# bernardomig/torch_semantic_segmentation

Hardware: AMD Instinct MI355X
Metric: images/sec (train step) fastscnn 1024x2048 bs=8 (higher is better)
Workload: dtype bf16; 1 GPU; fastscnn train step (zero_grad+fwd+CE(ignore 255)+bwd+AdamW), 8 x 3 x 1024 x 2048 per GPU, 19 classes, random-init weights; global_batch=8, parallelism=dp1, hip_graph=True, syncbn=False

## Files before the change

### torch_semantic_segmentation_amd/csrc/wgrad.hip

```cpp
#include "common.h"
#include "wgreduce.h"
#include "bnfin.h"

extern int g_tss_disable_fast;

namespace {

constexpr int TN = 128, TK = 128, NT = 256;
enum { A_PW = 0, A_TAPS = 1, A_STEM = 2 };

template <typename T> struct WMma;
template <> struct WMma<bf16_t> {
  static constexpr int PT = 64, KSTEP = 32;
  typedef bf16x8 Frag;
  static __device__ __forceinline__ Frag ld(const unsigned char* row, int swz, int ks, int q) {
    return *reinterpret_cast<const bf16x8*>(row + (((ks * 4 + q) ^ swz) << 4));
  }
  static __device__ __forceinline__ f32x4 mma(Frag a, Frag b, f32x4 c) {
    return __builtin_amdgcn_mfma_f32_16x16x32_bf16(a, b, c, 0, 0, 0);
  }
};
template <> struct WMma<float> {
  static constexpr int PT = 32, KSTEP = 4;
  typedef float Frag;
  static __device__ __forceinline__ Frag ld(const unsigned char* row, int swz, int ks, int q) {
    return *reinterpret_cast<const float*>(row + ((ks ^ swz) << 4) + q * 4);
  }
  static __device__ __forceinline__ f32x4 mma(Frag a, Frag b, f32x4 c) {
    return __builtin_amdgcn_mfma_f32_16x16x4f32(a, b, c, 0, 0, 0);
  }
};
constexpr int ROWB = 144;

struct WgradArgs {
  long P;
  int ND, KD, ntaps, mode;
  const void* e; long lde; const void* yraw; long ldyr;
  const float* ga; const float* gb; const float* gce; const float* gmu;
  const void* x; long ldx; const float* xm; const float* xs; const float* xb; int x_relu, x_f32;
  int Hin, Win, Hout, Wout, stride, dil, Cin;
  int tap0, tstep1;
  int gkh, gkw;
  float* dw; long drs, dcs, dts;
  int nsplit;
  float* ws;
  tss_bn_bwd_job fin; int fin_blocks;
};

template <typename T> struct Pack4;
template <> struct Pack4<bf16_t> {
  static __device__ __forceinline__ void put(unsigned char* dst, float a, float b, float c, float d) {
    bf16x4 o; o[0] = (bf16_t)a; o[1] = (bf16_t)b; o[2] = (bf16_t)c; o[3] = (bf16_t)d;
    *reinterpret_cast<bf16x4*>(dst) = o;
  }
};
template <> struct Pack4<float> {
  static __device__ __forceinline__ void put(unsigned char* dst, float a, float b, float c, float d) {
    *reinterpret_cast<float4*>(dst) = make_float4(a, b, c, d);
  }
};
template <typename T>
__device__ __forceinline__ unsigned char* unit_addr(unsigned char* tile, int row, int pg) {
  const int boff = pg * 4 * (int)sizeof(T);
  return tile + row * ROWB + ((((boff >> 4)) ^ ((row >> 3) & 7)) << 4) + (boff & 15);
}
template <typename T>
__device__ __forceinline__ void put_unit(unsigned char* tile, int ch0, int pg, const float v[4][8]) {
#pragma unroll
  for (int j = 0; j < 8; ++j) Pack4<T>::put(unit_addr<T>(tile, ch0 + j, pg), v[0][j], v[1][j], v[2][j], v[3][j]);
}

template <typename T>
__global__ __launch_bounds__(NT, 2) void wgrad_kernel(const WgradArgs g) {
  typedef WMma<T> M;
  constexpr int PT = M::PT, NPG = PT / 4;
  constexpr bool FOLD = sizeof(T) == 2;
  __shared__ __align__(16) unsigned char Gt[TN * ROWB];
  __shared__ __align__(16) unsigned char At[TK * ROWB];
  __shared__ __align__(16) float Cg[4][TN];
  __shared__ __align__(16) float Ca[3][TK];

  const int tid = threadIdx.x, lane = tid & 63, wave = tid >> 6;
  const int fr = lane & 15, fq = lane >> 4;
  const int wn = wave >> 1, wk = wave & 1;

  const int nchn = (g.ND + TN - 1) / TN, nchk = (g.KD + TK - 1) / TK;
  int bid = blockIdx.x;
  const int split = bid % g.nsplit; bid /= g.nsplit;
  const int nc = bid % nchn; bid /= nchn;
  const int kc = bid % nchk; bid /= nchk;
  const int tap = bid;

  const int n0 = nc * TN, k0 = kc * TK;
  const int ncw = (g.ND - n0 < TN) ? (g.ND - n0) : TN;
  const int kcw = (g.KD - k0 < TK) ? (g.KD - k0) : TK;
  const int nvn = (ncw + 7) >> 3, nvk = (kcw + 7) >> 3;
  int nfn = (ncw - wn * 64 + 15) >> 4; nfn = nfn < 0 ? 0 : (nfn > 4 ? 4 : nfn);
  int nfk = (kcw - wk * 64 + 15) >> 4; nfk = nfk < 0 ? 0 : (nfk > 4 ? 4 : nfk);

  const long nstage = (g.P + PT - 1) / PT;
  const long per = (nstage + g.nsplit - 1) / g.nsplit;
  const long s_begin = split * per;
  long s_end = s_begin + per;
  if (s_end > nstage) s_end = nstage;

  f32x4 acc[4][4];
#pragma unroll
  for (int i = 0; i < 4; ++i)
#pragma unroll
    for (int j = 0; j < 4; ++j) acc[i][j] = (f32x4){0.f, 0.f, 0.f, 0.f};

  for (int i = tid; i < TN * ROWB / 16; i += NT) {
    reinterpret_cast<uint4*>(Gt)[i] = make_uint4(0, 0, 0, 0);
    reinterpret_cast<uint4*>(At)[i] = make_uint4(0, 0, 0, 0);
  }
  for (int i = tid; i < TN; i += NT) {
    const bool in = i < ncw;
    Cg[0][i] = (in && g.ga) ? g.ga[n0 + i] : 1.f;
    Cg[1][i] = (in && g.yraw) ? g.gb[n0 + i] : 0.f;
    Cg[2][i] = (in && g.yraw) ? g.gce[n0 + i] : 0.f;
    Cg[3][i] = (in && g.yraw) ? g.gmu[n0 + i] : 0.f;
    const bool ik = i < kcw && g.mode != A_STEM;
    Ca[0][i] = (ik && g.xs && g.xm) ? g.xm[k0 + i] : 0.f;
    Ca[1][i] = (ik && g.xs) ? g.xs[k0 + i] : 1.f;
    Ca[2][i] = (ik && g.xs && g.xb) ? g.xb[k0 + i] : 0.f;
  }

  const T* e = reinterpret_cast<const T*>(g.e);
  const T* yr = reinterpret_cast<const T*>(g.yraw);
  const T* x = reinterpret_cast<const T*>(g.x);
  const long HWo = (long)g.Hout * g.Wout;
  int tdy, tdx;
  if (g.gkw > 0) { const int ty = tap / g.gkw; tdy = ty - (g.gkh >> 1); tdx = (tap - ty * g.gkw) - (g.gkw >> 1); }
  else { const int tgrid = g.tap0 + tap * (g.tstep1 + 1); const int ky = tgrid / 3; tdy = ky - 1; tdx = tgrid - ky * 3 - 1; }
  tdy *= g.dil; tdx *= g.dil;

  for (long s = s_begin; s < s_end; ++s) {
    const long p0 = s * PT;
    __syncthreads();
    for (int u = tid; u < NPG * nvn; u += NT) {
      const int pg = u / nvn, cv = u - pg * nvn;
      const int ch = n0 + cv * 8;
      float v[4][8];
      float ca[8], cb[8], cc[8], cm[8];
#pragma unroll
      for (int j = 0; j < 8; ++j) {
        ca[j] = Cg[0][cv * 8 + j]; cb[j] = Cg[1][cv * 8 + j]; cc[j] = Cg[2][cv * 8 + j]; cm[j] = Cg[3][cv * 8 + j];
        if (FOLD) cc[j] = -(ca[j] * cc[j]) - cb[j] * cm[j];
      }
#pragma unroll
      for (int i = 0; i < 4; ++i) {
        const long p = p0 + pg * 4 + i;
        const bool ok = p < g.P;
        const long pc = ok ? p : 0;
        float ev[8];
        V8<T>::load(e + pc * g.lde + ch, ev);
        if (yr) {
          float yv[8];
          V8<T>::load(yr + pc * g.ldyr + ch, yv);
#pragma unroll
          for (int j = 0; j < 8; ++j)
            v[i][j] = FOLD ? ca[j] * ev[j] + (cb[j] * yv[j] + cc[j]) : ca[j] * (ev[j] - cc[j]) + cb[j] * (yv[j] - cm[j]);
        } else {
#pragma unroll
          for (int j = 0; j < 8; ++j) v[i][j] = ca[j] * ev[j];
        }
#pragma unroll
        for (int j = 0; j < 8; ++j) if (!ok || ch + j >= g.ND) v[i][j] = 0.f;
      }
      put_unit<T>(Gt, cv * 8, pg, v);
    }
    if (g.mode == A_STEM) {
      const float* src32 = reinterpret_cast<const float*>(g.x);
      for (int u = tid; u < NPG * kcw; u += NT) {
        const int pg = u % NPG, j = u / NPG;
        const int c = j / 9, t9 = j - c * 9, sy = t9 / 3, sx = t9 - sy * 3;
        float v[4];
#pragma unroll
        for (int i = 0; i < 4; ++i) {
          const long p = p0 + pg * 4 + i;
          v[i] = 0.f;
          if (p < g.P) {
            const long b = p / HWo; const long rem = p - b * HWo;
            const int oy = (int)(rem / g.Wout), ox = (int)(rem - (long)oy * g.Wout);
            const int iy = oy * g.stride + (sy - 1) * g.dil, ix = ox * g.stride + (sx - 1) * g.dil;
            if (iy >= 0 && iy < g.Hin && ix >= 0 && ix < g.Win) {
              const long off = ((b * g.Cin + c) * g.Hin + iy) * (long)g.Win + ix;
              v[i] = g.x_f32 ? src32[off] : (float)x[off];
            }
          }
        }
        Pack4<T>::put(unit_addr<T>(At, j, pg), v[0], v[1], v[2], v[3]);
      }
    } else {
      for (int u = tid; u < NPG * nvk; u += NT) {
        const int pg = u / nvk, cv = u - pg * nvk;
        const int ch = k0 + cv * 8;
        float v[4][8];
        float cm[8], cs[8], cb[8];
#pragma unroll
        for (int j = 0; j < 8; ++j) {
          cm[j] = Ca[0][cv * 8 + j]; cs[j] = Ca[1][cv * 8 + j]; cb[j] = Ca[2][cv * 8 + j];
          if (FOLD) cb[j] -= cm[j] * cs[j];
        }
#pragma unroll
        for (int i = 0; i < 4; ++i) {
          const long p = p0 + pg * 4 + i;
          long q = -1;
          if (p < g.P) {
            if (g.mode == A_PW) {
              q = p;
            } else {
              const long b = p / HWo; const long rem = p - b * HWo;
              const int oy = (int)(rem / g.Wout), ox = (int)(rem - (long)oy * g.Wout);
              const int iy = oy * g.stride + tdy, ix = ox * g.stride + tdx;
              if (iy >= 0 && iy < g.Hin && ix >= 0 && ix < g.Win) q = (b * g.Hin + iy) * (long)g.Win + ix;
            }
          }
          float xv[8];
          V8<T>::load(x + (q >= 0 ? q : 0) * g.ldx + ch, xv);
          const float vlo = q >= 0 ? (g.x_relu ? 0.f : -TSS_INF) : 0.f, vhi = q >= 0 ? TSS_INF : 0.f;
#pragma unroll
          for (int j = 0; j < 8; ++j) {
            v[i][j] = clamp3(FOLD ? xv[j] * cs[j] + cb[j] : (xv[j] - cm[j]) * cs[j] + cb[j], vlo, vhi);
            if (ch + j >= g.KD) v[i][j] = 0.f;
          }
        }
        put_unit<T>(At, cv * 8, pg, v);
      }
    }
    __syncthreads();
    if (nfn > 0 && nfk > 0) {
      const unsigned char* grow = Gt + (wn * 64 + fr) * ROWB;
      const unsigned char* arow = At + (wk * 64 + fr) * ROWB;
#pragma unroll
      for (int ks = 0; ks < PT / M::KSTEP; ++ks) {
        typename M::Frag gf[4], af[4];
#pragma unroll
        for (int i = 0; i < 4; ++i) {
          gf[i] = M::ld(grow + i * 16 * ROWB, ((wn * 64 + i * 16 + fr) >> 3) & 7, ks, fq);
          af[i] = M::ld(arow + i * 16 * ROWB, ((wk * 64 + i * 16 + fr) >> 3) & 7, ks, fq);
        }
#pragma unroll
        for (int i = 0; i < 4; ++i)
#pragma unroll
          for (int j = 0; j < 4; ++j)
            if (i < nfn && j < nfk) acc[i][j] = M::mma(gf[i], af[j], acc[i][j]);
      }
    }
  }

  float* dwt = g.dw + tap * g.dts;
  if (s_begin < s_end) {
#pragma unroll
    for (int i = 0; i < 4; ++i)
#pragma unroll
      for (int j = 0; j < 4; ++j) {
        if (i < nfn && j < nfk) {
          const int k = k0 + wk * 64 + j * 16 + fr;
#pragma unroll
          for (int r = 0; r < 4; ++r) {
            const int n = n0 + wn * 64 + i * 16 + fq * 4 + r;
            if (n < g.ND && k < g.KD) atomicAdd(dwt + (long)n * g.drs + (long)k * g.dcs, acc[i][j][r]);
          }
        }
      }
  }
}

using tss_wg::ws_dim;

#ifdef TSS_TIMING
__device__ unsigned long long g_wg_timing[8];
#define TSS_T(var) unsigned long long var; asm volatile("s_memtime %0\n s_waitcnt lgkmcnt(0)" : "=s"(var) :: "memory")
#else
#define TSS_T(var)
#endif
template <int PT>
__global__ __launch_bounds__(NT, 2) void wgfast_kernel(const WgradArgs g) {
  typedef bf16_t T;
  constexpr int NPG = PT / 4, ROW = PT * 2 + 16, NKS = PT / 32;
  TSS_T(tks);
  extern __shared__ __align__(16) unsigned char smem[];
  unsigned char* Gt = smem;
  unsigned char* At = smem + TN * ROW;

  const int tid = threadIdx.x, lane = tid & 63, wave = tid >> 6;
  const int fr = lane & 15, fq = lane >> 4;

  if ((int)blockIdx.x < g.fin_blocks) { tss_fin::bn_bwd_finalize_block(g.fin, blockIdx.x); return; }
  const int nchn = (g.ND + TN - 1) / TN;
  int bid = (int)blockIdx.x - g.fin_blocks;
  const int split = bid % g.nsplit; bid /= g.nsplit;
  const int nc = bid % nchn; bid /= nchn;
  const int kc = bid;
  const int n0 = nc * TN, k0 = kc * TK;
  const int ncw = (g.ND - n0 < TN) ? (g.ND - n0) : TN;
  const int kcw = (g.KD - k0 < TK) ? (g.KD - k0) : TK;
  const int nvn = ncw >> 3, nvk = kcw >> 3;
  const int FN = (ncw + 15) >> 4, FK = (kcw + 15) >> 4;

  int ib = 0, jb = 0, cn = 4, ck = 4, ks0 = 0, ks1 = NKS;
  if (FN > 4 && FK > 4) { ib = 4 * (wave >> 1); jb = 4 * (wave & 1); }
  else {
    ks0 = (wave & 1) * (NKS / 2); ks1 = ks0 + NKS / 2;
    if (FN > 4) ib = 4 * (wave >> 1);
    else if (FK > 4) jb = 4 * (wave >> 1);
    else if (FN > 2) { ib = 2 * (wave >> 1); cn = 2; }
    else { jb = 2 * (wave >> 1); ck = 2; }
  }
  cn = FN - ib < cn ? FN - ib : cn; cn = cn < 0 ? 0 : cn;
  ck = FK - jb < ck ? FK - jb : ck; ck = ck < 0 ? 0 : ck;

  const long nstage = (g.P + PT - 1) / PT;
  const long per = (nstage + g.nsplit - 1) / g.nsplit;
  const long s_begin = split * per;
  long s_end = s_begin + per;
  if (s_end > nstage) s_end = nstage;

  f32x4 acc[4][4];
#pragma unroll
  for (int i = 0; i < 4; ++i)
#pragma unroll
    for (int j = 0; j < 4; ++j) acc[i][j] = (f32x4){0.f, 0.f, 0.f, 0.f};

  const int pgG = tid / nvn, cvG = tid - pgG * nvn;
  const int pgA = tid / nvk, cvA = tid - pgA * nvk;
  const bool onG = pgG < NPG, onA = pgA < NPG;
  const T* eg = reinterpret_cast<const T*>(g.e) + n0 + (onG ? cvG * 8 : 0);
  const T* yg = reinterpret_cast<const T*>(g.yraw) + n0 + (onG ? cvG * 8 : 0);
  const T* xg = reinterpret_cast<const T*>(g.x) + k0 + (onA ? cvA * 8 : 0);
  uint4 re[4], ry[4], rx[4];
  auto issue_g = [&](long s) {
    const long p0 = s * PT;
    if (onG) {
#pragma unroll
      for (int i = 0; i < 4; ++i) {
        const long p = p0 + pgG * 4 + i;
        const long pc = p < g.P ? p : 0;
        re[i] = *reinterpret_cast<const uint4*>(eg + pc * g.lde);
        ry[i] = *reinterpret_cast<const uint4*>(yg + pc * g.ldyr);
      }
    }
  };
  auto issue_a = [&](long s) {
    const long p0 = s * PT;
    if (onA) {
#pragma unroll
      for (int i = 0; i < 4; ++i) {
        const long p = p0 + pgA * 4 + i;
        const long pc = p < g.P ? p : 0;
        rx[i] = *reinterpret_cast<const uint4*>(xg + pc * g.ldx);
      }
    }
  };
  auto unit_ptr = [&](unsigned char* tile, int row, int pg) -> unsigned char* {
    const int boff = pg * 8;
    return tile + row * ROW + ((((boff >> 4)) ^ ((row >> 3) & 7)) << 4) + (boff & 15);
  };
  auto blo = [](uint32_t u) { return __uint_as_float(u << 16); };
  auto bhi = [](uint32_t u) { return __uint_as_float(u & 0xffff0000u); };

#ifdef TSS_TIMING
  unsigned long long tph[7] = {0, 0, 0, 0, 0, 0, 0};
#endif
  if (s_begin < s_end) { issue_g(s_begin); issue_a(s_begin); }

  for (int i = tid; i < TN * ROW / 16; i += NT) {
    reinterpret_cast<uint4*>(Gt)[i] = make_uint4(0, 0, 0, 0);
    reinterpret_cast<uint4*>(At)[i] = make_uint4(0, 0, 0, 0);
  }
  float ca[8], cb[8], cc[8], as[8], ab[8];
  {
    const int chn = n0 + (onG ? cvG * 8 : 0), chk = k0 + (onA ? cvA * 8 : 0);
    const float* pxs = g.xs ? g.xs : g.ga;
    const float* pxb = (g.xs && g.xb) ? g.xb : g.ga;
    const float* pxm = (g.xs && g.xm) ? g.xm : g.ga;
    const int cks = g.xs ? chk : 0;
    float vga[8], vgb[8], vce[8], vmu[8], vs[8], vb[8], vm[8];
#pragma unroll
    for (int h = 0; h < 8; h += 4) {
      V4<float>::load(g.ga + chn + h, vga + h); V4<float>::load(g.gb + chn + h, vgb + h);
      V4<float>::load(g.gce + chn + h, vce + h); V4<float>::load(g.gmu + chn + h, vmu + h);
      V4<float>::load(pxs + cks + h, vs + h); V4<float>::load(pxb + cks + h, vb + h); V4<float>::load(pxm + cks + h, vm + h);
    }
    const bool has_s = g.xs != nullptr, has_b = has_s && g.xb != nullptr, has_m = has_s && g.xm != nullptr;
#pragma unroll
    for (int j = 0; j < 8; ++j) {
      ca[j] = vga[j]; cb[j] = vgb[j]; cc[j] = -(vga[j] * vce[j]) - vgb[j] * vmu[j];
      const float sc = has_s ? vs[j] : 1.f;
      as[j] = sc; ab[j] = (has_b ? vb[j] : 0.f) - (has_m ? vm[j] : 0.f) * sc;
    }
  }
  const float relu_lo = g.x_relu ? 0.f : -TSS_INF;
  TSS_T(tk1);
#ifdef TSS_TIMING
  tph[5] += tk1 - tks;
#endif
  for (long s = s_begin; s < s_end; ++s) {
    const long p0 = s * PT;
    TSS_T(t0);
    __syncthreads();
    TSS_T(t1);
    if (onG) {
      float v[4][8];
#pragma unroll
      for (int i = 0; i < 4; ++i) {
        const bool ok = p0 + pgG * 4 + i < g.P;
        const uint32_t* ue = reinterpret_cast<const uint32_t*>(&re[i]);
        const uint32_t* uy = reinterpret_cast<const uint32_t*>(&ry[i]);
#pragma unroll
        for (int h = 0; h < 4; ++h) {
          v[i][2 * h] = ca[2 * h] * blo(ue[h]) + (cb[2 * h] * blo(uy[h]) + cc[2 * h]);
          v[i][2 * h + 1] = ca[2 * h + 1] * bhi(ue[h]) + (cb[2 * h + 1] * bhi(uy[h]) + cc[2 * h + 1]);
        }
        if (!ok) {
#pragma unroll
          for (int j = 0; j < 8; ++j) v[i][j] = 0.f;
        }
      }
#pragma unroll
      for (int j = 0; j < 8; ++j) Pack4<T>::put(unit_ptr(Gt, cvG * 8 + j, pgG), v[0][j], v[1][j], v[2][j], v[3][j]);
    }
    TSS_T(t2);
    if (s + 1 < s_end) issue_g(s + 1);
    if (onA) {
      float v[4][8];
#pragma unroll
      for (int i = 0; i < 4; ++i) {
        const bool ok = p0 + pgA * 4 + i < g.P;
        const uint32_t* ux = reinterpret_cast<const uint32_t*>(&rx[i]);
#pragma unroll
        for (int h = 0; h < 4; ++h) {
          v[i][2 * h] = fmaxf(blo(ux[h]) * as[2 * h] + ab[2 * h], relu_lo);
          v[i][2 * h + 1] = fmaxf(bhi(ux[h]) * as[2 * h + 1] + ab[2 * h + 1], relu_lo);
        }
        if (!ok) {
#pragma unroll
          for (int j = 0; j < 8; ++j) v[i][j] = 0.f;
        }
      }
#pragma unroll
      for (int j = 0; j < 8; ++j) Pack4<T>::put(unit_ptr(At, cvA * 8 + j, pgA), v[0][j], v[1][j], v[2][j], v[3][j]);
    }
    if (s + 1 < s_end) issue_a(s + 1);
    TSS_T(t3);
    __syncthreads();
    TSS_T(t4);

    if (cn > 0 && ck > 0) {
      const int rg = ib * 16 + fr, rk = jb * 16 + fr;
      const unsigned char* grow = Gt + rg * ROW;
      const unsigned char* arow = At + rk * ROW;
      for (int ks = ks0; ks < ks1; ++ks) {
        bf16x8 gf[4], af[4];
#pragma unroll
        for (int i = 0; i < 4; ++i) {
          if (i < cn) gf[i] = *reinterpret_cast<const bf16x8*>(grow + i * 16 * ROW + (((ks * 4 + fq) ^ (((rg + i * 16) >> 3) & 7)) << 4));
          if (i < ck) af[i] = *reinterpret_cast<const bf16x8*>(arow + i * 16 * ROW + (((ks * 4 + fq) ^ (((rk + i * 16) >> 3) & 7)) << 4));
        }
#pragma unroll
        for (int i = 0; i < 4; ++i)
#pragma unroll
          for (int j = 0; j < 4; ++j)
            if (i < cn && j < ck) acc[i][j] = __builtin_amdgcn_mfma_f32_16x16x32_bf16(gf[i], af[j], acc[i][j], 0, 0, 0);
      }
    }
    TSS_T(t5);
#ifdef TSS_TIMING
    tph[0] += t1 - t0; tph[1] += t2 - t1; tph[2] += t3 - t2; tph[3] += t4 - t3; tph[4] += t5 - t4;
#endif
  }

  TSS_T(tkl);
  if (g.ws) {
    const bool psplit = !(FN > 4 && FK > 4);
    if (psplit) {
      __syncthreads();
      f32x4* xch = reinterpret_cast<f32x4*>(smem) + (wave >> 1) * 16 * 64;
      if (wave & 1) {
#pragma unroll
        for (int i = 0; i < 4; ++i)
#pragma unroll
          for (int j = 0; j < 4; ++j)
            if (i < cn && j < ck) xch[(i * 4 + j) * 64 + lane] = acc[i][j];
      }
      __syncthreads();
      if (!(wave & 1)) {
#pragma unroll
        for (int i = 0; i < 4; ++i)
#pragma unroll
          for (int j = 0; j < 4; ++j)
            if (i < cn && j < ck) acc[i][j] += xch[(i * 4 + j) * 64 + lane];
      }
    }
    if (!psplit || !(wave & 1)) {
      const int tile = kc * nchn + nc;
      const int TNe = ws_dim(g.ND), TKe = ws_dim(g.KD);
      float* wt = g.ws + ((long)tile * g.nsplit + split) * (TNe * TKe);
#pragma unroll
      for (int i = 0; i < 4; ++i)
#pragma unroll
        for (int j = 0; j < 4; ++j) {
          if (i < cn && j < ck) {
            float* wf = wt + ((ib + i) * (TKe >> 4) + (jb + j)) * 256 + fq * 16 + fr;
#pragma unroll
            for (int r = 0; r < 4; ++r) wf[r * 64] = acc[i][j][r];
          }
        }
    }
  } else if (s_begin < s_end) {
#pragma unroll
    for (int i = 0; i < 4; ++i)
#pragma unroll
      for (int j = 0; j < 4; ++j) {
        if (i < cn && j < ck) {
          const int k = k0 + (jb + j) * 16 + fr;
#pragma unroll
          for (int r = 0; r < 4; ++r) {
            const int n = n0 + (ib + i) * 16 + fq * 4 + r;
            if (n < g.ND && k < g.KD) atomicAdd(g.dw + (long)n * g.drs + (long)k * g.dcs, acc[i][j][r]);
          }
        }
      }
  }
#ifdef TSS_TIMING
  asm volatile("s_waitcnt vmcnt(0)" ::: "memory");
  TSS_T(tk2);
  tph[6] = tk2 - tkl;
  if (threadIdx.x == 0) {
    for (int q = 0; q < 7; ++q) atomicAdd(&g_wg_timing[q], tph[q]);
    atomicAdd(&g_wg_timing[7], 1ull);
  }
#endif
}

__global__ __launch_bounds__(NT) void wg_reduce_kernel(const tss_wg::ReduceArgs r) {
  __shared__ float4 part[4 * 64];
  tss_wg::reduce_block(r, blockIdx.x, part);
}

using tss_wg::reduce_args;

template <int PT>
void launch_fast_pt(WgradArgs& g, hipStream_t stream, bool defer_reduce) {
  const tss_wg::Split sp = tss_wg::split_for(g.P, g.KD, g.ND);
  g.nsplit = sp.nsplit;
  constexpr int smem = 2 * TN * (PT * 2 + 16);
  static tss::DevOnce attr;
  if (attr.first()) {
    (void)hipFuncSetAttribute(reinterpret_cast<const void*>(wgfast_kernel<PT>), hipFuncAttributeMaxDynamicSharedMemorySize, smem);
  }
  hipLaunchKernelGGL(wgfast_kernel<PT>, dim3(sp.tiles * g.nsplit + g.fin_blocks), dim3(NT), smem, stream, g);
  if (g.ws && !defer_reduce) {
    const tss_wg::ReduceArgs r = reduce_args(g.ws, g.dw, g.P, g.KD, g.ND);
    hipLaunchKernelGGL(wg_reduce_kernel, dim3(r.nred), dim3(NT), 0, stream, r);
  }
}

int launch(WgradArgs& g, int dtype, int kernel_id, hipStream_t stream, double alg_bytes) {
  if (g.P <= 0) return TSS_OK;
  const int nchn = (g.ND + TN - 1) / TN, nchk = (g.KD + TK - 1) / TK;
  const int tiles = nchn * nchk * g.ntaps;
  const int PT = dtype == TSS_BF16 ? WMma<bf16_t>::PT : WMma<float>::PT;
  const long nstage = (g.P + PT - 1) / PT;
  constexpr long MIN_STAGES = 8;
  long ns = 1024 / tiles;
  if (ns < 1) ns = 1;
  if (ns > (nstage + MIN_STAGES - 1) / MIN_STAGES) ns = (nstage + MIN_STAGES - 1) / MIN_STAGES;
  if (ns < 1) ns = 1;
  g.nsplit = (int)ns;
  const int grid = tiles * (int)ns;
  tss::ProfScope prof(kernel_id, stream, alg_bytes, 2.0 * (double)g.P * g.ND * g.KD * g.ntaps);
  if (dtype == TSS_BF16) hipLaunchKernelGGL(wgrad_kernel<bf16_t>, dim3(grid), dim3(NT), 0, stream, g);
  else hipLaunchKernelGGL(wgrad_kernel<float>, dim3(grid), dim3(NT), 0, stream, g);
  return tss::check_last("wgrad");
}

}

bool tss_stem_direct_wgrad(const void* e, long lde, const void* yraw, long ldyr, const float* ga, const float* gb,
                           const float* gce, const float* gmu, const void* x_nchw, int x_is_f32, float* dw, float* ws,
                           int B, int Cin, int Hin, int Win, int N, int stride, int dtype, hipStream_t stream);

void tss_wg_reduce_standalone(const float* ws, float* dw, long P, int K, int N, hipStream_t stream) {
  const tss_wg::ReduceArgs r = reduce_args(ws, dw, P, K, N);
  hipLaunchKernelGGL(wg_reduce_kernel, dim3(r.nred), dim3(NT), 0, stream, r);
}

extern "C" {

int tss_pwconv_bwd_weight(const void* e, long lde, const void* yraw, long ldyr,
                          const float* ga, const float* gb, const float* gce, const float* gmu,
                          const void* xraw, long ldx, const float* in_mean, const float* in_scale, const float* in_bias, int in_relu,
                          float* dw, float* ws, int defer_reduce, long P, int K, int N, int dtype, const tss_bn_bwd_job* fin,
                          void* stream) {
  TSS_REQUIRE(dtype == TSS_F32 || dtype == TSS_BF16, TSS_ERR_DTYPE);
  TSS_REQUIRE(!fin || (fin->C > 0 && fin->count >= 1.0 && fin->bstats && fin->invstd && fin->ga && fin->gb && fin->gce), TSS_ERR_SHAPE);
  TSS_REQUIRE(K > 0 && N > 0 && (K % 8) == 0 && (lde % 8) == 0 && lde >= (N + 7) / 8 * 8 && (ldx % 8) == 0 && ldx >= K, TSS_ERR_SHAPE);
  TSS_REQUIRE(!yraw || ((ldyr % 8) == 0 && ldyr >= (N + 7) / 8 * 8 && ga && gb && gce && gmu), TSS_ERR_SHAPE);
  TSS_REQUIRE(tss::aligned16(e) && tss::aligned16(xraw), TSS_ERR_ALIGN);
  WgradArgs g = {};
  g.P = P; g.ND = N; g.KD = K; g.ntaps = 1; g.mode = A_PW;
  g.e = e; g.lde = lde; g.yraw = yraw; g.ldyr = ldyr; g.ga = ga; g.gb = gb; g.gce = gce; g.gmu = gmu;
  g.x = xraw; g.ldx = ldx; g.xm = in_mean; g.xs = in_scale; g.xb = in_bias; g.x_relu = in_relu;
  g.Hout = 1; g.Wout = 1;
  g.dw = dw; g.drs = K; g.dcs = 1; g.dts = 0;
  const double bytes = (double)P * (N * (yraw ? 2 : 1) + K) * tss::esz(dtype);
  if (dtype == TSS_BF16 && !g_tss_disable_fast && yraw && (N % 8) == 0 && P > 0) {
    tss::ProfScope prof(TSS_K_PWCONV_BWD_WEIGHT, (hipStream_t)stream, bytes, 2.0 * (double)P * N * K);
    g.ws = ws;
    if (fin) { g.fin = *fin; g.fin_blocks = tss_fin::fin_blocks(fin->C); }
    if (tss_wg::split_for(P, K, N).pt == 128) launch_fast_pt<128>(g, (hipStream_t)stream, ws && defer_reduce);
    else launch_fast_pt<64>(g, (hipStream_t)stream, ws && defer_reduce);
    return tss::check_last("wgfast");
  }
  if (fin) {
    const int rc = tss_bn_bwd_finalize(fin->bstats, fin->count, fin->invstd, fin->gamma, fin->training, fin->accumulate, fin->dgamma,
                                       fin->dbeta, fin->ga, fin->gb, fin->gce, fin->C, stream);
    if (rc != TSS_OK) return rc;
  }
  return launch(g, dtype, TSS_K_PWCONV_BWD_WEIGHT, (hipStream_t)stream, bytes);
}

int tss_pwconv_wg_reduce(const float* ws, float* dw, long P, int K, int N, void* stream) {
  TSS_REQUIRE(ws && dw && P > 0 && K > 0 && N > 0 && (K % 8) == 0 && (N % 8) == 0, TSS_ERR_SHAPE);
  tss_wg_reduce_standalone(ws, dw, P, K, N, (hipStream_t)stream);
  return tss::check_last("wg_reduce");
}

long tss_pwconv_bwd_weight_ws(long P, int K, int N, int dtype) {
  if (dtype != TSS_BF16 || g_tss_disable_fast || (N % 8) != 0 || (K % 8) != 0 || P <= 0) return 0;
  const tss_wg::Split sp = tss_wg::split_for(P, K, N);
  return (long)sp.tiles * sp.nsplit * ws_dim(N) * ws_dim(K);
}

int tss_conv3x3_bwd_weight(const void* e, long lde, const void* yraw, long ldyr,
                           const float* ga, const float* gb, const float* gce, const float* gmu,
                           const void* xraw, long ldx, const float* in_mean, const float* in_scale, const float* in_bias, int in_relu,
                           float* dw, int B, int Hin, int Win, int Cin, int N, int stride, int dil,
                           int dtype, void* stream) {
  TSS_REQUIRE(dtype == TSS_F32 || dtype == TSS_BF16, TSS_ERR_DTYPE);
  TSS_REQUIRE(Cin > 0 && N > 0 && (Cin % 8) == 0 && (N % 8) == 0 && (lde % 8) == 0 && lde >= N && (ldx % 8) == 0 && ldx >= Cin,
              TSS_ERR_SHAPE);
  TSS_REQUIRE(!yraw || ((ldyr % 8) == 0 && ldyr >= N && ga && gb && gce && gmu), TSS_ERR_SHAPE);
  WgradArgs g = {};
  g.Hin = Hin; g.Win = Win; g.stride = stride; g.dil = dil; g.Cin = Cin;
  g.Hout = (Hin - 1) / stride + 1; g.Wout = (Win - 1) / stride + 1;
  g.P = (long)B * g.Hout * g.Wout; g.ND = N; g.KD = Cin; g.ntaps = 9; g.mode = A_TAPS;
  g.e = e; g.lde = lde; g.yraw = yraw; g.ldyr = ldyr; g.ga = ga; g.gb = gb; g.gce = gce; g.gmu = gmu;
  g.x = xraw; g.ldx = ldx; g.xm = in_mean; g.xs = in_scale; g.xb = in_bias; g.x_relu = in_relu;
  g.dw = dw; g.drs = (long)Cin * 9; g.dcs = 9; g.dts = 1;
  return launch(g, dtype, TSS_K_CONV3X3_BWD_WEIGHT, (hipStream_t)stream,
                ((double)g.P * N * (yraw ? 2 : 1) + (double)B * Hin * Win * Cin) * tss::esz(dtype));
}

int tss_conv1d3_bwd_weight(const void* e, long lde, const void* yraw, long ldyr,
                           const float* ga, const float* gb, const float* gce, const float* gmu,
                           const void* xraw, long ldx, const float* in_mean, const float* in_scale, const float* in_bias, int in_relu,
                           float* dw, int B, int H, int W, int Cin, int N, int axis, int dil, int dtype, void* stream) {
  TSS_REQUIRE(dtype == TSS_F32 || dtype == TSS_BF16, TSS_ERR_DTYPE);
  TSS_REQUIRE(Cin > 0 && N > 0 && (Cin % 8) == 0 && (N % 8) == 0 && (lde % 8) == 0 && lde >= N && (ldx % 8) == 0 && ldx >= Cin &&
              (axis == 0 || axis == 1) && dil >= 1, TSS_ERR_SHAPE);
  TSS_REQUIRE(!yraw || ((ldyr % 8) == 0 && ldyr >= N && ga && gb && gce && gmu), TSS_ERR_SHAPE);
  WgradArgs g = {};
  g.Hin = H; g.Win = W; g.stride = 1; g.dil = dil; g.Cin = Cin; g.Hout = H; g.Wout = W;
  g.tap0 = axis == 0 ? 3 : 1; g.tstep1 = axis == 0 ? 0 : 2;
  g.P = (long)B * H * W; g.ND = N; g.KD = Cin; g.ntaps = 3; g.mode = A_TAPS;
  g.e = e; g.lde = lde; g.yraw = yraw; g.ldyr = ldyr; g.ga = ga; g.gb = gb; g.gce = gce; g.gmu = gmu;
  g.x = xraw; g.ldx = ldx; g.xm = in_mean; g.xs = in_scale; g.xb = in_bias; g.x_relu = in_relu;
  g.dw = dw; g.drs = (long)Cin * 3; g.dcs = 3; g.dts = 1;
  return launch(g, dtype, TSS_K_CONV3X3_BWD_WEIGHT, (hipStream_t)stream,
                ((double)g.P * N * (yraw ? 2 : 1) + (double)g.P * Cin) * tss::esz(dtype));
}

int tss_convkxk_bwd_weight(const void* e, long lde, const void* yraw, long ldyr,
                           const float* ga, const float* gb, const float* gce, const float* gmu,
                           const void* xraw, long ldx, const float* in_mean, const float* in_scale, const float* in_bias, int in_relu,
                           float* dw, int B, int Hin, int Win, int Cin, int N, int kh, int kw, int stride, int dil,
                           int dtype, void* stream) {
  TSS_REQUIRE(dtype == TSS_F32 || dtype == TSS_BF16, TSS_ERR_DTYPE);
  TSS_REQUIRE(Cin > 0 && N > 0 && (Cin % 8) == 0 && (N % 8) == 0 && (lde % 8) == 0 && lde >= N && (ldx % 8) == 0 && ldx >= Cin &&
              stride >= 1 && dil >= 1 && kh >= 1 && kw >= 1 && (kh & 1) && (kw & 1) && kh * kw <= 81, TSS_ERR_SHAPE);
  TSS_REQUIRE(!yraw || ((ldyr % 8) == 0 && ldyr >= N && ga && gb && gce && gmu), TSS_ERR_SHAPE);
  WgradArgs g = {};
  g.Hin = Hin; g.Win = Win; g.stride = stride; g.dil = dil; g.Cin = Cin; g.gkh = kh; g.gkw = kw;
  g.Hout = (Hin - 1) / stride + 1; g.Wout = (Win - 1) / stride + 1;
  g.P = (long)B * g.Hout * g.Wout; g.ND = N; g.KD = Cin; g.ntaps = kh * kw; g.mode = A_TAPS;
  g.e = e; g.lde = lde; g.yraw = yraw; g.ldyr = ldyr; g.ga = ga; g.gb = gb; g.gce = gce; g.gmu = gmu;
  g.x = xraw; g.ldx = ldx; g.xm = in_mean; g.xs = in_scale; g.xb = in_bias; g.x_relu = in_relu;
  g.dw = dw; g.drs = (long)Cin * kh * kw; g.dcs = kh * kw; g.dts = 1;
  return launch(g, dtype, TSS_K_CONV3X3_BWD_WEIGHT, (hipStream_t)stream,
                ((double)g.P * N * (yraw ? 2 : 1) + (double)B * Hin * Win * Cin) * tss::esz(dtype));
}

int tss_stem3x3_bwd_weight(const void* e, long lde, const void* yraw, long ldyr,
                           const float* ga, const float* gb, const float* gce, const float* gmu,
                           const void* x_nchw, int x_is_f32, float* dw, float* ws,
                           int B, int Cin, int Hin, int Win, int N, int stride, int dtype, void* stream) {
  TSS_REQUIRE(dtype == TSS_F32 || dtype == TSS_BF16, TSS_ERR_DTYPE);
  TSS_REQUIRE(Cin >= 1 && Cin * 9 <= TK && N > 0 && (N % 8) == 0 && (lde % 8) == 0 && lde >= N, TSS_ERR_SHAPE);
  TSS_REQUIRE(!yraw || ((ldyr % 8) == 0 && ldyr >= N && ga && gb && gce && gmu), TSS_ERR_SHAPE);
  WgradArgs g = {};
  g.Hin = Hin; g.Win = Win; g.stride = stride; g.dil = 1; g.Cin = Cin;
  g.Hout = (Hin - 1) / stride + 1; g.Wout = (Win - 1) / stride + 1;
  g.P = (long)B * g.Hout * g.Wout; g.ND = N; g.KD = Cin * 9; g.ntaps = 1; g.mode = A_STEM;
  g.e = e; g.lde = lde; g.yraw = yraw; g.ldyr = ldyr; g.ga = ga; g.gb = gb; g.gce = gce; g.gmu = gmu;
  g.x = x_nchw; g.x_f32 = x_is_f32;
  g.dw = dw; g.drs = (long)Cin * 9; g.dcs = 1; g.dts = 0;
  const double bytes = (double)g.P * N * (yraw ? 2 : 1) * tss::esz(dtype) + (double)B * Cin * Hin * Win * (x_is_f32 ? 4 : tss::esz(dtype));
  if (dtype == TSS_BF16 && !g_tss_disable_fast && Cin <= 3 && N == 32 && ws) {
    tss::ProfScope prof(TSS_K_STEM_BWD_WEIGHT, (hipStream_t)stream, bytes, 2.0 * (double)g.P * N * Cin * 9);
    if (tss_stem_direct_wgrad(e, lde, yraw, ldyr, ga, gb, gce, gmu, x_nchw, x_is_f32, dw, ws, B, Cin, Hin, Win, N, stride,
                              dtype, (hipStream_t)stream))
      return tss::check_last("stem_direct_wgrad");
  }
  return launch(g, dtype, TSS_K_STEM_BWD_WEIGHT, (hipStream_t)stream, bytes);
}

#ifdef TSS_TIMING
int tss_debug_wg_timing(unsigned long long* out8, int reset) {
  if (hipMemcpyFromSymbol(out8, HIP_SYMBOL(g_wg_timing), sizeof(unsigned long long) * 8) != hipSuccess) return -1;
  if (reset) { unsigned long long z[8] = {0}; (void)hipMemcpyToSymbol(HIP_SYMBOL(g_wg_timing), z, sizeof(z)); }
  return 0;
}
#endif

}
```

Before: 1721 images/sec.

## Restructure wgrad fast kernel with row-major staging, transpose LDS reads and double buffering

Rewrites the pointwise-conv weight-gradient fast kernel. Threads now load whole rows and store them into a double-buffered LDS image, and MFMA operands come from transposed LDS reads (tr_pair). This replaces the old per-thread 4-pixel transpose-on-store into a single buffer. The kernel is fixed to 64-pixel sub-stages that iterate within the split's stage range, which removes the PT=128 variant. It also uses 32-bit unsigned offsets, so it adds a leading-dimension guard and falls back to the generic path when strides are large. The aim is fewer barriers per stage and cheaper LDS writes, at the cost of more shared memory and extra code from the template specialisations.

New measurement: 1728 images/sec (median of 6 runs). About the same (+0.4%).

```diff
diff --git a/torch_semantic_segmentation_amd/csrc/wgrad.hip b/torch_semantic_segmentation_amd/csrc/wgrad.hip
--- a/torch_semantic_segmentation_amd/csrc/wgrad.hip
+++ b/torch_semantic_segmentation_amd/csrc/wgrad.hip
@@ -1,5 +1,6 @@
 #include "common.h"
 #include "wgreduce.h"
+#include "wgsweep.h"
 #include "bnfin.h"
 
 extern int g_tss_disable_fast;
@@ -42,7 +43,7 @@
   int tap0, tstep1;
   int gkh, gkw;
   float* dw; long drs, dcs, dts;
-  int nsplit;
+  int nsplit, pt;
   float* ws;
   tss_bn_bwd_job fin; int fin_blocks;
 };
@@ -276,16 +277,20 @@
 #else
 #define TSS_T(var)
 #endif
+template <int N> struct IntC { static constexpr int value = N; };
+
 template <int PT>
 __global__ __launch_bounds__(NT, 2) void wgfast_kernel(const WgradArgs g) {
   typedef bf16_t T;
-  constexpr int NPG = PT / 4, ROW = PT * 2 + 16, NKS = PT / 32;
+  static_assert(PT == 64, "one 16-chunk plane of 64 rows per operand, two k-steps");
+  constexpr int IMG = PT * 256, BUF = 2 * IMG;
   TSS_T(tks);
   extern __shared__ __align__(16) unsigned char smem[];
-  unsigned char* Gt = smem;
-  unsigned char* At = smem + TN * ROW;
-
-  const int tid = threadIdx.x, lane = tid & 63, wave = tid >> 6;
+  float* Cg = reinterpret_cast<float*>(smem + 2 * BUF);
+  float* Ca = Cg + 16 * 24;
+
+  const int tid = threadIdx.x, lane = tid & 63;
+  const int wave = __builtin_amdgcn_readfirstlane(tid >> 6);
   const int fr = lane & 15, fq = lane >> 4;
 
   if ((int)blockIdx.x < g.fin_blocks) { tss_fin::bn_bwd_finalize_block(g.fin, blockIdx.x); return; }
@@ -300,10 +305,10 @@
   const int nvn = ncw >> 3, nvk = kcw >> 3;
   const int FN = (ncw + 15) >> 4, FK = (kcw + 15) >> 4;
 
-  int ib = 0, jb = 0, cn = 4, ck = 4, ks0 = 0, ks1 = NKS;
+  int ib = 0, jb = 0, cn = 4, ck = 4, ks0 = 0, ks1 = 2;
   if (FN > 4 && FK > 4) { ib = 4 * (wave >> 1); jb = 4 * (wave & 1); }
   else {
-    ks0 = (wave & 1) * (NKS / 2); ks1 = ks0 + NKS / 2;
+    ks0 = wave & 1; ks1 = ks0 + 1;
     if (FN > 4) ib = 4 * (wave >> 1);
     else if (FK > 4) jb = 4 * (wave >> 1);
     else if (FN > 2) { ib = 2 * (wave >> 1); cn = 2; }
@@ -312,11 +317,14 @@
   cn = FN - ib < cn ? FN - ib : cn; cn = cn < 0 ? 0 : cn;
   ck = FK - jb < ck ? FK - jb : ck; ck = ck < 0 ? 0 : ck;
 
-  const long nstage = (g.P + PT - 1) / PT;
+  const long nstage = (g.P + g.pt - 1) / g.pt;
   const long per = (nstage + g.nsplit - 1) / g.nsplit;
   const long s_begin = split * per;
   long s_end = s_begin + per;
   if (s_end > nstage) s_end = nstage;
+  const long q_begin = s_begin * (g.pt / PT);
+  long q_end = s_end * (g.pt / PT);
+  if (q_end > (g.P + PT - 1) / PT) q_end = (g.P + PT - 1) / PT;
 
   f32x4 acc[4][4];
 #pragma unroll
@@ -324,152 +332,122 @@
 #pragma unroll
     for (int j = 0; j < 4; ++j) acc[i][j] = (f32x4){0.f, 0.f, 0.f, 0.f};
 
-  const int pgG = tid / nvn, cvG = tid - pgG * nvn;
-  const int pgA = tid / nvk, cvA = tid - pgA * nvk;
-  const bool onG = pgG < NPG, onA = pgA < NPG;
-  const T* eg = reinterpret_cast<const T*>(g.e) + n0 + (onG ? cvG * 8 : 0);
-  const T* yg = reinterpret_cast<const T*>(g.yraw) + n0 + (onG ? cvG * 8 : 0);
-  const T* xg = reinterpret_cast<const T*>(g.x) + k0 + (onA ? cvA * 8 : 0);
-  uint4 re[4], ry[4], rx[4];
-  auto issue_g = [&](long s) {
-    const long p0 = s * PT;
-    if (onG) {
-#pragma unroll
-      for (int i = 0; i < 4; ++i) {
-        const long p = p0 + pgG * 4 + i;
-        const long pc = p < g.P ? p : 0;
-        re[i] = *reinterpret_cast<const uint4*>(eg + pc * g.lde);
-        ry[i] = *reinterpret_cast<const uint4*>(yg + pc * g.ldyr);
-      }
+  const int rpG = NT / nvn, rpA = NT / nvk;
+  const int cvG = tid % nvn, rowG = tid / nvn, cvA = tid % nvk, rowA = tid / nvk;
+  const bool onG = rowG < rpG, onA = rowA < rpA;
+  const unsigned offE = (unsigned)(rowG * (int)g.lde + cvG * 8) * 2u, offY = (unsigned)(rowG * (int)g.ldyr + cvG * 8) * 2u;
+  const unsigned offX = (unsigned)(rowA * (int)g.ldx + cvA * 8) * 2u;
+  const unsigned stepE = (unsigned)(rpG * (int)g.lde) * 2u, stepY = (unsigned)(rpG * (int)g.ldyr) * 2u, stepX = (unsigned)(rpA * (int)g.ldx) * 2u;
+  const unsigned char* eb = reinterpret_cast<const unsigned char*>(reinterpret_cast<const T*>(g.e) + n0);
+  const unsigned char* yb = reinterpret_cast<const unsigned char*>(reinterpret_cast<const T*>(g.yraw) + n0);
+  const unsigned char* xb = reinterpret_cast<const unsigned char*>(reinterpret_cast<const T*>(g.x) + k0);
+
+  int troffG[4][2], troffA[4][2];
+#pragma unroll
+  for (int i = 0; i < 4; ++i)
+#pragma unroll
+    for (int h = 0; h < 2; ++h) {
+      troffG[i][h] = wgs::tr_off(PT, fr, fq, h, (ib + i) & 7);
+      troffA[i][h] = IMG + wgs::tr_off(PT, fr, fq, h, (jb + i) & 7);
     }
+
+  wgs::Fold<true> f;
+  auto sweep = [&](auto npg_c, auto npa_c) {
+    constexpr int NPG = decltype(npg_c)::value, NPA = decltype(npa_c)::value;
+    uint4 re[NPG], ry[NPG], rx[NPA];
+    auto rows_of = [&](long q) -> int { const long left = g.P - q * PT; return left < PT ? (int)left : PT; };
+    auto issue_g = [&](long q) {
+      const int lim = rows_of(q);
+      const unsigned char* be = eb + q * PT * g.lde * 2;
+      const unsigned char* by = yb + q * PT * g.ldyr * 2;
+#pragma unroll
+      for (int p = 0; p < NPG; ++p) {
+        const bool ok = rowG + p * rpG < lim;
+        re[p] = *reinterpret_cast<const uint4*>(be + (ok ? offE + p * stepE : (unsigned)cvG * 16u));
+        ry[p] = *reinterpret_cast<const uint4*>(by + (ok ? offY + p * stepY : (unsigned)cvG * 16u));
+      }
+    };
+    auto issue_a = [&](long q) {
+      const int lim = rows_of(q);
+      const unsigned char* bx = xb + q * PT * g.ldx * 2;
+#pragma unroll
+      for (int p = 0; p < NPA; ++p) {
+        const bool ok = rowA + p * rpA < lim;
+        rx[p] = *reinterpret_cast<const uint4*>(bx + (ok ? offX + p * stepX : (unsigned)cvA * 16u));
+      }
+    };
+    issue_g(q_begin); issue_a(q_begin);
+    {
+      wgs::Operands o = {};
+      o.e = reinterpret_cast<const T*>(g.e); o.y = reinterpret_cast<const T*>(g.yraw);
+      o.ga = g.ga; o.gb = g.gb; o.gce = g.gce; o.gmu = g.gmu;
+      o.xs = g.xs; o.xm = g.xs ? g.xm : nullptr; o.xb = g.xs ? g.xb : nullptr; o.x_relu = g.x_relu;
+      f.load(o, n0 + cvG * 8, k0 + cvA * 8);
+    }
+    if (rowG == 0) { V8<float>::store(Cg + cvG * 24, f.ca); V8<float>::store(Cg + cvG * 24 + 8, f.cb); V8<float>::store(Cg + cvG * 24 + 16, f.cc); }
+    if (rowA == 0) { V8<float>::store(Ca + cvA * 16, f.as); V8<float>::store(Ca + cvA * 16 + 8, f.ab); }
+    if (tid < 2 * PT) {
+      const int row = tid & (PT - 1);
+      unsigned char* img = smem + (tid >> 6) * BUF;
+      if (nvn & 1) *reinterpret_cast<uint4*>(img + img_off(row, nvn)) = make_uint4(0u, 0u, 0u, 0u);
+      if (nvk & 1) *reinterpret_cast<uint4*>(img + IMG + img_off(row, nvk)) = make_uint4(0u, 0u, 0u, 0u);
+    }
+    __syncthreads();
+    int b = 0;
+    auto stage = [&](long q, auto more_c) {
+      constexpr bool MORE = decltype(more_c)::value != 0;
+      unsigned char* img = smem + b * BUF;
+      const int lim = rows_of(q);
+      V8<float>::load(Cg + cvG * 24, f.ca); V8<float>::load(Cg + cvG * 24 + 8, f.cb); V8<float>::load(Cg + cvG * 24 + 16, f.cc);
+#pragma unroll
+      for (int p = 0; p < NPG; ++p) {
+        const int row = rowG + p * rpG;
+        const uint4 o = wgs::g_row<true>(re[p], ry[p], f, row < lim);
+        if (onG && row < PT) *reinterpret_cast<uint4*>(img + img_off(row, cvG)) = o;
+      }
+      if (MORE) issue_g(q + 1);
+      V8<float>::load(Ca + cvA * 16, f.as); V8<float>::load(Ca + cvA * 16 + 8, f.ab);
+#pragma unroll
+      for (int p = 0; p < NPA; ++p) {
+        const int row = rowA + p * rpA;
+        const uint4 o = wgs::a_row<true>(rx[p], f, row < lim);
+        if (onA && row < PT) *reinterpret_cast<uint4*>(img + IMG + img_off(row, cvA)) = o;
+      }
+      if (MORE) issue_a(q + 1);
+      __syncthreads();
+      if (cn > 0 && ck > 0) {
+#pragma unroll
+        for (int ks = 0; ks < 2; ++ks) {
+          if (ks >= ks0 && ks < ks1) {
+            const unsigned char* base = img + ks * 32 * 256;
+            bf16x8 af[4];
+#pragma unroll
+            for (int j = 0; j < 4; ++j)
+              if (j < ck) af[j] = tr_pair(base + troffA[j][0], base + troffA[j][1]);
+#pragma unroll
+            for (int i = 0; i < 4; ++i) {
+              if (i < cn) {
+                const bf16x8 gf = tr_pair(base + troffG[i][0], base + troffG[i][1]);
+#pragma unroll
+                for (int j = 0; j < 4; ++j)
+                  if (j < ck) acc[i][j] = __builtin_amdgcn_mfma_f32_16x16x32_bf16(gf, af[j], acc[i][j], 0, 0, 0);
+              }
+            }
+          }
+        }
+      }
+      b ^= 1;
+    };
+    long q = q_begin;
+    for (; q + 1 < q_end; ++q) stage(q, IntC<1>());
+    stage(q, IntC<0>());
   };
-  auto issue_a = [&](long s) {
-    const long p0 = s * PT;
-    if (onA) {
-#pragma unroll
-      for (int i = 0; i < 4; ++i) {
-        const long p = p0 + pgA * 4 + i;
-        const long pc = p < g.P ? p : 0;
-        rx[i] = *reinterpret_cast<const uint4*>(xg + pc * g.ldx);
-      }
-    }
-  };
-  auto unit_ptr = [&](unsigned char* tile, int row, int pg) -> unsigned char* {
-    const int boff = pg * 8;
-    return tile + row * ROW + ((((boff >> 4)) ^ ((row >> 3) & 7)) << 4) + (boff & 15);
-  };
-  auto blo = [](uint32_t u) { return __uint_as_float(u << 16); };
-  auto bhi = [](uint32_t u) { return __uint_as_float(u & 0xffff0000u); };
-
-#ifdef TSS_TIMING
-  unsigned long long tph[7] = {0, 0, 0, 0, 0, 0, 0};
-#endif
-  if (s_begin < s_end) { issue_g(s_begin); issue_a(s_begin); }
-
-  for (int i = tid; i < TN * ROW / 16; i += NT) {
-    reinterpret_cast<uint4*>(Gt)[i] = make_uint4(0, 0, 0, 0);
-    reinterpret_cast<uint4*>(At)[i] = make_uint4(0, 0, 0, 0);
-  }
-  float ca[8], cb[8], cc[8], as[8], ab[8];
-  {
-    const int chn = n0 + (onG ? cvG * 8 : 0), chk = k0 + (onA ? cvA * 8 : 0);
-    const float* pxs = g.xs ? g.xs : g.ga;
-    const float* pxb = (g.xs && g.xb) ? g.xb : g.ga;
-    const float* pxm = (g.xs && g.xm) ? g.xm : g.ga;
-    const int cks = g.xs ? chk : 0;
-    float vga[8], vgb[8], vce[8], vmu[8], vs[8], vb[8], vm[8];
-#pragma unroll
-    for (int h = 0; h < 8; h += 4) {
-      V4<float>::load(g.ga + chn + h, vga + h); V4<float>::load(g.gb + chn + h, vgb + h);
-      V4<float>::load(g.gce + chn + h, vce + h); V4<float>::load(g.gmu + chn + h, vmu + h);
-      V4<float>::load(pxs + cks + h, vs + h); V4<float>::load(pxb + cks + h, vb + h); V4<float>::load(pxm + cks + h, vm + h);
-    }
-    const bool has_s = g.xs != nullptr, has_b = has_s && g.xb != nullptr, has_m = has_s && g.xm != nullptr;
-#pragma unroll
-    for (int j = 0; j < 8; ++j) {
-      ca[j] = vga[j]; cb[j] = vgb[j]; cc[j] = -(vga[j] * vce[j]) - vgb[j] * vmu[j];
-      const float sc = has_s ? vs[j] : 1.f;
-      as[j] = sc; ab[j] = (has_b ? vb[j] : 0.f) - (has_m ? vm[j] : 0.f) * sc;
-    }
-  }
-  const float relu_lo = g.x_relu ? 0.f : -TSS_INF;
+
   TSS_T(tk1);
-#ifdef TSS_TIMING
-  tph[5] += tk1 - tks;
-#endif
-  for (long s = s_begin; s < s_end; ++s) {
-    const long p0 = s * PT;
-    TSS_T(t0);
-    __syncthreads();
-    TSS_T(t1);
-    if (onG) {
-      float v[4][8];
-#pragma unroll
-      for (int i = 0; i < 4; ++i) {
-        const bool ok = p0 + pgG * 4 + i < g.P;
-        const uint32_t* ue = reinterpret_cast<const uint32_t*>(&re[i]);
-        const uint32_t* uy = reinterpret_cast<const uint32_t*>(&ry[i]);
-#pragma unroll
-        for (int h = 0; h < 4; ++h) {
-          v[i][2 * h] = ca[2 * h] * blo(ue[h]) + (cb[2 * h] * blo(uy[h]) + cc[2 * h]);
-          v[i][2 * h + 1] = ca[2 * h + 1] * bhi(ue[h]) + (cb[2 * h + 1] * bhi(uy[h]) + cc[2 * h + 1]);
-        }
-        if (!ok) {
-#pragma unroll
-          for (int j = 0; j < 8; ++j) v[i][j] = 0.f;
-        }
-      }
-#pragma unroll
-      for (int j = 0; j < 8; ++j) Pack4<T>::put(unit_ptr(Gt, cvG * 8 + j, pgG), v[0][j], v[1][j], v[2][j], v[3][j]);
-    }
-    TSS_T(t2);
-    if (s + 1 < s_end) issue_g(s + 1);
-    if (onA) {
-      float v[4][8];
-#pragma unroll
-      for (int i = 0; i < 4; ++i) {
-        const bool ok = p0 + pgA * 4 + i < g.P;
-        const uint32_t* ux = reinterpret_cast<const uint32_t*>(&rx[i]);
-#pragma unroll
-        for (int h = 0; h < 4; ++h) {
-          v[i][2 * h] = fmaxf(blo(ux[h]) * as[2 * h] + ab[2 * h], relu_lo);
-          v[i][2 * h + 1] = fmaxf(bhi(ux[h]) * as[2 * h + 1] + ab[2 * h + 1], relu_lo);
-        }
-        if (!ok) {
-#pragma unroll
-          for (int j = 0; j < 8; ++j) v[i][j] = 0.f;
-        }
-      }
-#pragma unroll
-      for (int j = 0; j < 8; ++j) Pack4<T>::put(unit_ptr(At, cvA * 8 + j, pgA), v[0][j], v[1][j], v[2][j], v[3][j]);
-    }
-    if (s + 1 < s_end) issue_a(s + 1);
-    TSS_T(t3);
-    __syncthreads();
-    TSS_T(t4);
-
-    if (cn > 0 && ck > 0) {
-      const int rg = ib * 16 + fr, rk = jb * 16 + fr;
-      const unsigned char* grow = Gt + rg * ROW;
-      const unsigned char* arow = At + rk * ROW;
-      for (int ks = ks0; ks < ks1; ++ks) {
-        bf16x8 gf[4], af[4];
-#pragma unroll
-        for (int i = 0; i < 4; ++i) {
-          if (i < cn) gf[i] = *reinterpret_cast<const bf16x8*>(grow + i * 16 * ROW + (((ks * 4 + fq) ^ (((rg + i * 16) >> 3) & 7)) << 4));
-          if (i < ck) af[i] = *reinterpret_cast<const bf16x8*>(arow + i * 16 * ROW + (((ks * 4 + fq) ^ (((rk + i * 16) >> 3) & 7)) << 4));
-        }
-#pragma unroll
-        for (int i = 0; i < 4; ++i)
-#pragma unroll
-          for (int j = 0; j < 4; ++j)
-            if (i < cn && j < ck) acc[i][j] = __builtin_amdgcn_mfma_f32_16x16x32_bf16(gf[i], af[j], acc[i][j], 0, 0, 0);
-      }
-    }
-    TSS_T(t5);
-#ifdef TSS_TIMING
-    tph[0] += t1 - t0; tph[1] += t2 - t1; tph[2] += t3 - t2; tph[3] += t4 - t3; tph[4] += t5 - t4;
-#endif
+  if (q_begin < q_end) {
+    const bool g4 = 2 * rpG < PT, a4 = 2 * rpA < PT;
+    if (g4) { if (a4) sweep(IntC<4>(), IntC<4>()); else sweep(IntC<4>(), IntC<2>()); }
+    else { if (a4) sweep(IntC<2>(), IntC<4>()); else sweep(IntC<2>(), IntC<2>()); }
   }
 
   TSS_T(tkl);
@@ -509,7 +487,7 @@
           }
         }
     }
-  } else if (s_begin < s_end) {
+  } else if (q_begin < q_end) {
 #pragma unroll
     for (int i = 0; i < 4; ++i)
 #pragma unroll
@@ -527,9 +505,10 @@
 #ifdef TSS_TIMING
   asm volatile("s_waitcnt vmcnt(0)" ::: "memory");
   TSS_T(tk2);
-  tph[6] = tk2 - tkl;
   if (threadIdx.x == 0) {
-    for (int q = 0; q < 7; ++q) atomicAdd(&g_wg_timing[q], tph[q]);
+    atomicAdd(&g_wg_timing[4], tkl - tk1);
+    atomicAdd(&g_wg_timing[5], tk1 - tks);
+    atomicAdd(&g_wg_timing[6], tk2 - tkl);
     atomicAdd(&g_wg_timing[7], 1ull);
   }
 #endif
@@ -542,16 +521,11 @@
 
 using tss_wg::reduce_args;
 
-template <int PT>
-void launch_fast_pt(WgradArgs& g, hipStream_t stream, bool defer_reduce) {
+void launch_fast(WgradArgs& g, hipStream_t stream, bool defer_reduce) {
   const tss_wg::Split sp = tss_wg::split_for(g.P, g.KD, g.ND);
-  g.nsplit = sp.nsplit;
-  constexpr int smem = 2 * TN * (PT * 2 + 16);
-  static tss::DevOnce attr;
-  if (attr.first()) {
-    (void)hipFuncSetAttribute(reinterpret_cast<const void*>(wgfast_kernel<PT>), hipFuncAttributeMaxDynamicSharedMemorySize, smem);
-  }
-  hipLaunchKernelGGL(wgfast_kernel<PT>, dim3(sp.tiles * g.nsplit + g.fin_blocks), dim3(NT), smem, stream, g);
+  g.nsplit = sp.nsplit; g.pt = sp.pt;
+  constexpr int smem = 2 * 2 * 64 * 256 + 16 * 40 * 4;
+  wgs::launch_with_smem<wgfast_kernel<64>>(sp.tiles * g.nsplit + g.fin_blocks, NT, smem, stream, g);
   if (g.ws && !defer_reduce) {
     const tss_wg::ReduceArgs r = reduce_args(g.ws, g.dw, g.P, g.KD, g.ND);
     hipLaunchKernelGGL(wg_reduce_kernel, dim3(r.nred), dim3(NT), 0, stream, r);
@@ -607,12 +581,11 @@
   g.Hout = 1; g.Wout = 1;
   g.dw = dw; g.drs = K; g.dcs = 1; g.dts = 0;
   const double bytes = (double)P * (N * (yraw ? 2 : 1) + K) * tss::esz(dtype);
-  if (dtype == TSS_BF16 && !g_tss_disable_fast && yraw && (N % 8) == 0 && P > 0) {
+  if (dtype == TSS_BF16 && !g_tss_disable_fast && yraw && (N % 8) == 0 && P > 0 && lde < (1L << 20) && ldyr < (1L << 20) && ldx < (1L << 20)) {
     tss::ProfScope prof(TSS_K_PWCONV_BWD_WEIGHT, (hipStream_t)stream, bytes, 2.0 * (double)P * N * K);
     g.ws = ws;
     if (fin) { g.fin = *fin; g.fin_blocks = tss_fin::fin_blocks(fin->C); }
-    if (tss_wg::split_for(P, K, N).pt == 128) launch_fast_pt<128>(g, (hipStream_t)stream, ws && defer_reduce);
-    else launch_fast_pt<64>(g, (hipStream_t)stream, ws && defer_reduce);
+    launch_fast(g, (hipStream_t)stream, ws && defer_reduce);
     return tss::check_last("wgfast");
   }
   if (fin) {
```
